# kureta/ddsp-pytorch

Measured on AMD Instinct MI355X. Metric: audio samples/sec/GPU + %HBM-roofline, 16kHz/100-harmonic/batch512, higher is better.
Workload: dtype f32

## Files before the change

ddsp-pytorch_amd/_lib.py:

```python
from __future__ import annotations

import ctypes
import os
import subprocess

_DIR = os.path.dirname(os.path.abspath(__file__))
SO_PATH = os.environ.get("DDSP_HIP_LIB", os.path.join(_DIR, "libddsp_hip.so"))
ABI_VERSION = 5

_lib = None


class DdspHipError(RuntimeError):
    pass


def build(force: bool = False, jobs: int = 4) -> str:
    args = ["make", "-C", os.path.join(_DIR, "csrc"), f"-j{jobs}"]
    if force:
        args.append("-B")
    r = subprocess.run(args, capture_output=True, text=True)
    if r.returncode != 0:
        raise DdspHipError("building libddsp_hip.so failed:\n" + r.stdout[-4000:] + r.stderr[-4000:])
    return SO_PATH


_vp, _i32, _u32, _u64, _long, _size, _f32, _f64 = (ctypes.c_void_p, ctypes.c_int, ctypes.c_uint, ctypes.c_uint64, ctypes.c_long,
                                                   ctypes.c_size_t, ctypes.c_float, ctypes.c_double)

SIGNATURES = {
    "ddsp_hip_abi_version": (_i32, []),
    "ddsp_test_hooks_enabled": (_i32, []),
    "ddsp_osc_scratch_bytes": (_size, [_i32, _i32, _i32]),
    "ddsp_osc_forward_ex": (_i32, [_vp] * 8 + [_i32] * 5 + [_u32, _vp]),
    "ddsp_noise_workspace_bytes": (_size, [_i32, _i32, _i32, _i32]),
    "ddsp_noise_forward_ws": (_i32, [_vp, _vp, _vp, _i32, _i32, _i32, _i32, _u64, _u64, _vp, _i32, _vp, _size, _vp]),
    "ddsp_noise_backward_ws": (_i32, [_vp, _vp, _vp, _i32, _i32, _i32, _i32, _u64, _u64, _vp, _vp, _size, _vp]),
    "ddsp_noise_ola_workspace_bytes": (_size, [_i32, _i32, _i32, _i32]),
    "ddsp_noise_ola_forward": (_i32, [_vp, _vp, _vp, _i32, _i32, _i32, _i32, _u64, _u64, _vp, _i32, _vp, _size, _vp]),
    "ddsp_noise_ola_backward": (_i32, [_vp, _vp, _vp, _i32, _i32, _i32, _i32, _u64, _u64, _vp, _vp, _size, _vp]),
    "ddsp_noise_ola_stream_state_floats": (_size, [_i32]),
    "ddsp_noise_ola_stream": (_i32, [_vp] * 6 + [_i32, _i32, _i32, _i32, _u64, _u64, _vp, _vp, _size, _vp]),
    "ddsp_osc_backward_scratch_bytes": (_size, [_i32, _i32, _i32]),
    "ddsp_osc_backward": (_i32, [_vp] * 8 + [_i32] * 5 + [_vp]),
    "ddsp_osc_set_tiling": (_i32, [_i32]),
    "ddsp_osc_set_path": (_i32, [_i32]),
    "ddsp_osc_plan": (_i32, [_i32] * 5 + [ctypes.POINTER(_i32), _i32]),
    "ddsp_osc_clock": (_i32, [_vp, _i32, _i32, _i32, _i32, _i32, ctypes.POINTER(ctypes.c_double), _vp]),
    "ddsp_noise_set_residency": (_i32, [_i32]),
    "ddsp_noise_get_residency": (_i32, []),
    "ddsp_noise_set_generic": (_i32, [_i32]),
    "ddsp_profile_enable": (_i32, [_i32]),
    "ddsp_profile_select": (_i32, [_u32]),
    "ddsp_profile_read": (_i32, [ctypes.POINTER(_i32), ctypes.POINTER(_f32), _i32]),
    "ddsp_gru_scratch_bytes": (_size, [_i32, _i32]),
    "ddsp_gru_max_batch": (_i32, [_i32, _i32]),
    "ddsp_gru_forward": (_i32, [_vp] * 9 + [_i32] * 3 + [_vp]),
    "ddsp_gru_backward": (_i32, [_vp] * 11 + [_i32] * 3 + [_vp]),
    "ddsp_gru_status": (_i32, [_vp, ctypes.POINTER(_i32)]),
    "ddsp_gru_forward_bf16": (_i32, [_vp] * 9 + [_i32] * 3 + [_vp]),
    "ddsp_gru_backward_bf16": (_i32, [_vp] * 11 + [_i32] * 4 + [_vp]),
    "ddsp_gru_set_mode": (_i32, [_i32]),
    "ddsp_gru_set_fault_step": (_i32, [_i32]),
    "ddsp_outer_ln_lrelu_scratch_bytes": (_size, [_i32]),
    "ddsp_outer_ln_lrelu_forward": (_i32, [_vp] * 8 + [_long, _i32, _f32, _f32, _i32, _vp]),
    "ddsp_outer_ln_lrelu_backward": (_i32, [_vp] * 13 + [_long, _i32, _f32, _i32, _vp]),
    "ddsp_colsum_scratch_bytes": (_size, [_i32]),
    "ddsp_colsum": (_i32, [_vp, _vp, _vp, _long, _i32, _i32, _vp]),
    "ddsp_stft_frames": (_i32, [_vp, _vp, _vp, _long, _long, _i32, _i32, _vp]),
    "ddsp_stft_frames_backward": (_i32, [_vp, _vp, _vp, _long, _long, _i32, _i32, _i32, _vp]),
    "ddsp_mss_scale_scratch_bytes": (_size, []),
    "ddsp_mss_scale_supported": (_i32, [_i32]),
    "ddsp_mss_scale": (_i32, [_vp] * 6 + [_long, _long, _i32, _i32, _f32, _f32, _vp]),
    "ddsp_reverb_impulse": (_i32, [_vp] * 5 + [_i32, _i32, _vp]),
    "ddsp_reverb_impulse_backward": (_i32, [_vp] * 8 + [_i32, _i32, _vp]),
    "ddsp_spectral_mul": (_i32, [_vp, _vp, _vp, _long, _long, _vp]),
    "ddsp_spectral_mul_backward": (_i32, [_vp] * 5 + [_long, _long, _vp]),
    "ddsp_reverb_live_scratch_bytes": (_size, [_i32, _i32]),
    "ddsp_reverb_live": (_i32, [_vp] * 9 + [_i32, _i32, _vp]),
    "ddsp_spectral_loss_scratch_bytes": (_size, []),
    "ddsp_spectral_loss": (_i32, [_vp] * 5 + [_long, _f32, _f32, _vp]),
    "ddsp_scaled_sigmoid_forward": (_i32, [_vp, _vp, _long, _vp]),
    "ddsp_scaled_sigmoid_backward": (_i32, [_vp, _vp, _vp, _long, _vp]),
    "ddsp_heads_sigmoid_forward": (_i32, [_vp] * 4 + [_long, _i32, _i32, _i32, _i32, _vp]),
    "ddsp_heads_sigmoid_backward": (_i32, [_vp] * 5 + [_long, _i32, _i32, _i32, _i32, _vp]),
    "ddsp_ln_lrelu_scratch_bytes": (_size, [_i32]),
    "ddsp_ln_lrelu_forward": (_i32, [_vp] * 6 + [_long, _i32, _f32, _f32, _vp]),
    "ddsp_ln_lrelu_backward": (_i32, [_vp] * 11 + [_long, _i32, _f32, _vp]),
    "ddsp_ln_lrelu_forward_16": (_i32, [_vp] * 6 + [_long, _i32, _f32, _f32, _i32, _vp]),
    "ddsp_ln_lrelu_backward_16": (_i32, [_vp] * 11 + [_long, _i32, _f32, _i32, _vp]),
    "ddsp_resample": (_i32, [_vp] * 4 + [_long, _long, _i32, _i32, _i32, _vp]),
    "ddsp_crepe_frames": (_i32, [_vp] * 3 + [_long, _long, _i32, _long, _vp]),
    "ddsp_crepe_epilogue": (_i32, [_vp] * 7 + [_long, _i32, _i32, _i32, _vp]),
    "ddsp_pitch_decode": (_i32, [_vp] * 8 + [_long, _vp]),
    "ddsp_pitch_centered": (_i32, [_vp] * 6 + [_long, _vp]),
    "ddsp_pitch_viterbi_workspace_bytes": (_size, [_long, _long]),
    "ddsp_pitch_viterbi": (_i32, [_vp] * 6 + [_long, _long, _vp]),
    "ddsp_pitch_voicing_workspace_bytes": (_size, [_long, _long]),
    "ddsp_pitch_voicing": (_i32, [_vp] * 11 + [_long, _long, _i32, _i32, _f32, _f32, _f32, _i32, _vp]),
    "ddsp_yin_salience": (_i32, [_vp] * 3 + [_long, _long, _i32, _long, _vp]),
    "ddsp_harm_workspace_bytes": (_size, [_long, _long, _i32]),
    "ddsp_harm_analysis": (_i32, [_vp] * 7 + [_long, _long, _i32, _i32, _i32, _i32, _vp]),
    "ddsp_harm_resynth": (_i32, [_vp] * 6 + [_long, _long, _i32, _i32, _i32, _u32, _vp]),
    "ddsp_harm_refine_workspace_bytes": (_size, [_long, _long, _i32]),
    "ddsp_harm_refine": (_i32, [_vp] * 8 + [_long, _long, _i32, _i32, _i32, _i32, _f32, _u32, _vp]),
    "ddsp_noise_analysis_workspace_bytes": (_size, [_long, _long, _i32, _i32]),
    "ddsp_noise_analysis": (_i32, [_vp] * 4 + [_long, _long, _i32, _i32, _i32, _i32, _vp]),
    "ddsp_noise_analysis_ola_workspace_bytes": (_size, [_long, _long, _i32, _i32]),
    "ddsp_noise_analysis_ola": (_i32, [_vp] * 4 + [_long, _long, _i32, _i32, _i32, _i32, _vp]),
    "ddsp_transform_controls": (_i32, [_vp] * 11 + [_long, _long, _long, _i32, _i32, _i32, _i32, _vp]),
    "ddsp_morph_controls": (_i32, [_vp] * 17 + [_long, _long, _long, _long, _i32, _i32, _i32, _i32, _i32, _i32, _vp]),
    "ddsp_dtw_workspace_bytes": (_size, [_long, _long, _long]),
    "ddsp_dtw_align": (_i32, [_vp] * 8 + [_size, _long, _long, _long, _i32, _long, _long, _f32, _f64, _vp]),
    "ddsp_loudness_supported": (_i32, [_i32]),
    "ddsp_loudness": (_i32, [_vp] * 3 + [_long, _long, _i32, _i32, _vp]),
    "ddsp_pcm_to_mono": (_i32, [_vp, _vp, _long, _i32, _i32, _vp]),
    "ddsp_make_examples": (_i32, [_vp, _long, _vp, _i32, _long, _long, _long, _long, _i32, _vp, _vp, _vp]),
    "ddsp_griffinlim_supported": (_i32, [_i32]),
    "ddsp_griffinlim_workspace_bytes": (_size, [_long, _long, _i32, _i32]),
    "ddsp_griffinlim": (_i32, [_vp] * 6 + [_size, _long, _long, _i32, _i32, _long, _i32, _f32, _vp]),
    "ddsp_wfft_probe_sizes": (_i32, [_i32, _long, ctypes.POINTER(_long), ctypes.POINTER(_long)]),
    "ddsp_wfft_probe": (_i32, [_i32, _vp, _vp, _long, _vp]),
    "ddsp_griffinlim_stage": (_i32, [_i32] + [_vp] * 8 + [_long, _long, _i32, _i32, _long, _f32, _vp]),
    "ddsp_gather_batch": (_i32, [_vp, _vp, ctypes.POINTER(_long), _i32, _vp, _vp, _long, _long, _i32, _i32, _vp, _vp]),
}
EXPORTS = tuple(SIGNATURES)


def lib():
    global _lib
    if _lib is not None:
        return _lib
    if not os.path.exists(SO_PATH):
        raise DdspHipError(
            f"{SO_PATH} is missing: the DDSP hot path has no CPU fallback. "
            "Build it with `python -c 'import __graft_entry__ as g; g.build()'` or `make -C ddsp-pytorch_amd/csrc`.")
    L = ctypes.CDLL(SO_PATH)
    abi = L.ddsp_hip_abi_version()
    if abi != ABI_VERSION:
        raise DdspHipError(f"{SO_PATH} has ABI {abi}, expected {ABI_VERSION}: rebuild "
                           "(`make -C ddsp-pytorch_amd/csrc` or __graft_entry__.build())")
    for name, (restype, argtypes) in SIGNATURES.items():
        fn = getattr(L, name)
        fn.restype, fn.argtypes = restype, argtypes
    _lib = L
    return L


KERNEL_NAMES = {1: "osc_frame_totals", 2: "osc_scan", 3: "osc_frame_synth", 4: "noise_frame", 5: "noise_impulse_responses"}


def profile_enable(capacity: int, only=None) -> None:
    mask = 0
    for name in only or ():
        mask |= 1 << [k for k, v in KERNEL_NAMES.items() if v == name][0]
    check(lib().ddsp_profile_select(mask), "ddsp_profile_select")
    check(lib().ddsp_profile_enable(capacity), "ddsp_profile_enable")


def profile_read(cap: int = 65536):
    ids = (ctypes.c_int * cap)()
    ms = (ctypes.c_float * cap)()
    n = lib().ddsp_profile_read(ids, ms, cap)
    return [(KERNEL_NAMES.get(ids[i], str(ids[i])), float(ms[i])) for i in range(n)]


def check(rc: int, what: str) -> None:
    if rc == 0:
        return
    if rc == -1:
        raise DdspHipError(f"{what}: invalid argument (DDSP_EINVAL)")
    if rc == -2:
        raise DdspHipError(f"{what}: shape outside the supported range (DDSP_ERANGE)")
    if rc == -3:
        raise DdspHipError(f"{what}: test / tuning hook refused (DDSP_EPERM): set DDSP_TEST_HOOKS=1 before the library is loaded")
    raise DdspHipError(f"{what}: HIP error {rc}")


def osc_plan(B: int, T: int, H: int, hop: int, sample_rate: int) -> dict:
    out = (ctypes.c_int * 8)()
    check(lib().ddsp_osc_plan(B, T, H, hop, sample_rate, out, 8), "ddsp_osc_plan")
    keys = ("harmonics_per_lane", "lanes_per_row", "chunked", "chunk_samples", "chunks_per_row", "row_blocks",
            "compute_units", "workgroups_per_unit")
    return dict(zip(keys, list(out)))


def osc_clock(scratch, B: int, T: int, H: int, hop: int, sample_rate: int, stream: int = 0) -> float:
    ghz = ctypes.c_double(0.0)
    check(lib().ddsp_osc_clock(scratch.data_ptr(), B, T, H, hop, sample_rate, ctypes.byref(ghz), stream or None), "ddsp_osc_clock")
    return float(ghz.value)
```

ddsp-pytorch_amd/csrc/ddsp_noise_wave.hip:

```cpp
#include <hip/hip_runtime.h>
#include <stdint.h>

#include <atomic>

#include "ddsp_hip.h"
#include "ddsp_internal.h"
#include "ddsp_noise_common.h"

using namespace ddsp_noise;

namespace {

typedef float v4f __attribute__((ext_vector_type(4)));

struct Tile { v4f v[5]; };
struct Lines { v4f v[8]; };
struct Pass { float v[16]; };
struct Spectra { v4f e[2], o[2], h64; float z32; };

constexpr int R = kWaveHop;
constexpr int F = kWaveBands;
constexpr int FG = kWaveGroupFrames;
static_assert(R == 128 && F == 65 && FG == 16 && 2 * (F - 1) == R, "the kernel's register and LDS layouts are written for these");
constexpr int KS = 132;
constexpr int XS = 140;
constexpr int kLdsFloats = FG * KS + FG * XS;

#ifndef DDSP_NOISE_ABL
#define DDSP_NOISE_ABL 0
#endif

#ifdef DDSP_NOISE_STAMPS
#define DDSP_STAMP(i) do { asm volatile("s_waitcnt lgkmcnt(0)" ::: "memory"); const unsigned long long now_ = __builtin_amdgcn_s_memtime(); \
                           stamp_sum[i] += now_ - stamp_last; stamp_last = now_; } while (0)
#else
#define DDSP_STAMP(i) do { } while (0)
#endif

template <bool ACC>
__global__ void __launch_bounds__(64, 2) noise_wave_kernel(NoiseParams p, long ngroups)
{
    extern __shared__ __attribute__((aligned(16))) float smem[];
    float *kern = smem;
    float *xs = smem + FG * KS;
    float *Hs = kern, *ys = xs;
    const int lane = threadIdx.x;
#ifdef DDSP_NOISE_STAMPS
    unsigned long long stamp_sum[8] = {0, 0, 0, 0, 0, 0, 0, 0}, stamp_last = __builtin_amdgcn_s_memtime();
    unsigned long long *stamp_out = reinterpret_cast<unsigned long long *>(const_cast<float *>(p.u)) + 8 * blockIdx.x;
    p.u = nullptr;
#endif

    const int mi0 = lane & 15, mq0 = lane >> 4;
    float *ctab = xs;
    ctab[lane] = cospif((float)lane * (1.0f / 64.0f));
    ctab[lane + 64] = cospif((float)(lane + 64) * (1.0f / 64.0f));
    DDSP_WAVE_ORDER();
    Split Be[2], Bo[2];
#pragma unroll
    for (int t = 0; t < 2; ++t) {
        const int n = 16 * t + mi0;
#pragma unroll
        for (int j = 0; j < 8; ++j) {
            const int k = 8 * mq0 + j;
            split3((k == 0 ? 0.5f : 1.0f) * ctab[(2 * k * n) & 127], Be[t], j);
            split3(ctab[((2 * k + 1) * n) & 127], Bo[t], j);
        }
    }
    float w1[2], w2[2];
#pragma unroll
    for (int t = 0; t < 2; ++t) {
        const int n = 16 * t + mi0;
        w1[t] = __fmaf_rn(0.5f, ctab[n], 0.5f) * (1.0f / 64.0f);
        w2[t] = __fmaf_rn(0.5f, ctab[64 - n], 0.5f) * (1.0f / 64.0f);
    }
    DDSP_WAVE_ORDER();
    const uint64_t base_off = p.offset + (p.offset_dev ? *p.offset_dev : 0ull);

    auto load_tile = [&](long g) {
        const v4f *src = reinterpret_cast<const v4f *>(p.Hm + g * FG * F);
        Tile h;
#pragma unroll
        for (int j = 0; j < 4; ++j) h.v[j] = src[lane + 64 * j];
        h.v[4] = src[256 + (lane & 3)];
        return h;
    };

    auto opaque_lane = [&]() { int ln = lane; asm volatile("" : "+v"(ln)); return ln; };

    auto products = [&](const Tile h) {
        const int ln = opaque_lane(), mi = ln & 15, mq = ln >> 4;
#pragma unroll
        for (int j = 0; j < 4; ++j) *reinterpret_cast<v4f *>(Hs + 4 * (ln + 64 * j)) = h.v[j];
        if (ln < 4) *reinterpret_cast<v4f *>(Hs + 4 * (ln + 256)) = h.v[4];
        DDSP_WAVE_ORDER();
        const float *hrow = Hs + mi * F + 16 * mq;
        float hv[16];
#pragma unroll
        for (int j = 0; j < 16; ++j) hv[j] = hrow[j];
        const float h64 = Hs[mi * F + 64];
        Spectra sp;
#pragma unroll
        for (int r = 0; r < 4; ++r) sp.h64[r] = 0.5f * Hs[(4 * mq + r) * F + 64];
        DDSP_WAVE_ORDER();
        Split Ae, Ao;
#pragma unroll
        for (int j = 0; j < 8; ++j) { split3(hv[2 * j], Ae, j); split3(hv[2 * j + 1], Ao, j); }
        v4f (&accE)[2] = sp.e, (&accO)[2] = sp.o;
        accE[0] = accE[1] = accO[0] = accO[1] = (v4f){0, 0, 0, 0};
        constexpr int PA[6] = {2, 1, 0, 1, 0, 0}, PB[6] = {0, 1, 2, 0, 1, 0};
#pragma unroll
        for (int i = 0; i < (DDSP_NOISE_ABL == 3 ? 1 : 6); ++i) {
            accE[0] = __builtin_amdgcn_mfma_f32_16x16x32_bf16(Ae.p[PA[i]], Be[0].p[PB[i]], accE[0], 0, 0, 0);
            accE[1] = __builtin_amdgcn_mfma_f32_16x16x32_bf16(Ae.p[PA[i]], Be[1].p[PB[i]], accE[1], 0, 0, 0);
            accO[0] = __builtin_amdgcn_mfma_f32_16x16x32_bf16(Ao.p[PA[i]], Bo[0].p[PB[i]], accO[0], 0, 0, 0);
            accO[1] = __builtin_amdgcn_mfma_f32_16x16x32_bf16(Ao.p[PA[i]], Bo[1].p[PB[i]], accO[1], 0, 0, 0);
        }
        float t = (mq == 0 ? 0.5f : 1.0f) * hv[0];
#pragma unroll
        for (int j = 1; j < 8; ++j) t += (j & 1) ? -hv[2 * j] : hv[2 * j];
        t += __shfl_xor(t, 16);
        t += __shfl_xor(t, 32);
        sp.z32 = (t + 0.5f * h64) * (0.5f / 64.0f);
        return sp;
    };

    auto taps = [&](const Spectra sp) {
        const int ln = opaque_lane(), mi = ln & 15, mq = ln >> 4;
        const v4f (&accE)[2] = sp.e, (&accO)[2] = sp.o;
        const float z32 = sp.z32;
#pragma unroll
        for (int t = 0; t < 2; ++t) {
            const int n = 16 * t + mi;
#pragma unroll
            for (int r = 0; r < 4; ++r) {
                float *kr = kern + (4 * mq + r) * KS;
                const float ev = accE[t][r] + ((mi & 1) ? -sp.h64[r] : sp.h64[r]);
                const float v1 = (ev + accO[t][r]) * w1[t];
                const float v2 = (ev - accO[t][r]) * w2[t];
                kr[n] = v1;
                if (n != 0) { kr[128 - n] = v1; kr[64 - n] = v2; }
                kr[64 + n] = v2;
            }
        }
        if (mq == 0) { kern[mi * KS + 32] = z32; kern[mi * KS + 96] = z32; }
        DDSP_WAVE_ORDER();
    };

    auto draw = [&](long frame0) {
        const int ln = opaque_lane();
        for (int e = ln; e < FG * 8; e += 64) xs[(e >> 3) * XS + (e & 7)] = 0.0f;
        if (p.u) {
#pragma unroll
            for (int j = 0; j < 8; ++j) {
                const int qi = ln + 64 * j, fr = qi >> 5, q = qi & 31;
                float4 v = *reinterpret_cast<const float4 *>(p.u + (frame0 + fr) * R + 4 * q);
                v.x = v.x * 2.0f - 1.0f; v.y = v.y * 2.0f - 1.0f; v.z = v.z * 2.0f - 1.0f; v.w = v.w * 2.0f - 1.0f;
                *reinterpret_cast<float4 *>(xs + fr * XS + 8 + 4 * q) = v;
            }
        } else {
            const uint64_t c0 = base_off + (uint64_t)frame0 * 32u + (uint64_t)ln;
#pragma unroll
            for (int j = 0; j < 8; ++j) {
                const int qi = ln + 64 * j, fr = qi >> 5, q = qi & 31;
                const uint64_t ctr = c0 + 64u * j;
                uint32_t rr[4];
                if (DDSP_NOISE_ABL == 2) { rr[0] = (uint32_t)ctr; rr[1] = rr[0] * 3u; rr[2] = rr[0] ^ 77u; rr[3] = rr[0] + 5u; }
                else philox4x32_10((uint32_t)ctr, (uint32_t)(ctr >> 32), (uint32_t)p.seed, (uint32_t)(p.seed >> 32), rr);
                float4 v;
                v.x = philox_to_sample(rr[0]); v.y = philox_to_sample(rr[1]); v.z = philox_to_sample(rr[2]); v.w = philox_to_sample(rr[3]);
                *reinterpret_cast<float4 *>(xs + fr * XS + 8 + 4 * q) = v;
            }
        }
        DDSP_WAVE_ORDER();
    };

    auto conv_pass = [&](int pass) {
        const int ln = opaque_lane();
        const int l5 = ln & 31, seg = l5 >> 2;
        const int cf = ((seg >> 1) << 2) | (l5 & 3);
        const int cs = 2 * (ln >> 5) + ((0x96 >> seg) & 1);
        const float *krow = kern + cf * KS;
        const float *xrow = xs + cf * XS + 8;
        const int cA = pass ? 8 + cs : 15 - cs, cB = 15 - cA;
        const int tsw = cA + 1;
        const float *kq_a = krow, *kq_b = krow - 8 * tsw;
        const float *xq_a = xrow + 8 * cA - 8 - 128, *xq_b = xrow + 8 * cB - 8 + 8 * tsw - 128;
        float acc[8], first[8];
#pragma unroll
        for (int u = 0; u < 8; ++u) { acc[u] = 0.0f; first[u] = 0.0f; }
        float4 cur[6], nxt[6];
        auto fetch = [&](float4 (&d)[6], const float *kq, const float *xq, int t) {
            d[0] = *reinterpret_cast<const float4 *>(kq + 8 * t);
            d[1] = *reinterpret_cast<const float4 *>(kq + 8 * t + 4);
            d[2] = *reinterpret_cast<const float4 *>(xq + 8 * (16 - t));
            d[3] = *reinterpret_cast<const float4 *>(xq + 8 * (16 - t) + 4);
            d[4] = *reinterpret_cast<const float4 *>(xq + 8 * (16 - t) + 8);
            d[5] = *reinterpret_cast<const float4 *>(xq + 8 * (16 - t) + 12);
        };
        fetch(cur, kq_a, xq_a, 0);
#pragma unroll
        for (int t = 0; t < (DDSP_NOISE_ABL == 1 ? 1 : 17); ++t) {
            if (t < 16) {
                if (t + 1 < 9) fetch(nxt, kq_a, xq_a, t + 1);
                else { const bool b = t + 1 >= tsw; fetch(nxt, b ? kq_b : kq_a, b ? xq_b : xq_a, t + 1); }
            }
            if (t >= 9 && t == tsw) {
                asm volatile("" ::: "memory");
#pragma unroll
                for (int u = 0; u < 8; ++u) { first[u] = acc[u]; acc[u] = 0.0f; }
            }
            asm volatile("" ::"v"(cur[2].x));
            const float kv[8] = {cur[0].x, cur[0].y, cur[0].z, cur[0].w, cur[1].x, cur[1].y, cur[1].z, cur[1].w};
            const float xw[16] = {cur[2].x, cur[2].y, cur[2].z, cur[2].w, cur[3].x, cur[3].y, cur[3].z, cur[3].w,
                                  cur[4].x, cur[4].y, cur[4].z, cur[4].w, cur[5].x, cur[5].y, cur[5].z, cur[5].w};
#pragma unroll
            for (int v = 0; v < 8; ++v)
#pragma unroll
                for (int u = 0; u < 8; ++u) acc[u] = __fmaf_rn(kv[v], xw[8 + u - v], acc[u]);
#pragma unroll
            for (int e = 0; e < 6; ++e) cur[e] = nxt[e];
            __builtin_amdgcn_sched_barrier(0);
        }
        Pass out;
#pragma unroll
        for (int u = 0; u < 8; ++u) { out.v[u] = first[u]; out.v[8 + u] = acc[u]; }
        return out;
    };

    auto stage = [&](const Pass r0, const Pass r1) {
        const int ln = opaque_lane();
        const int l5 = ln & 31, seg = l5 >> 2;
        const int cf = ((seg >> 1) << 2) | (l5 & 3);
        const int cs = 2 * (ln >> 5) + ((0x96 >> seg) & 1);
        DDSP_WAVE_ORDER();
#pragma unroll
        for (int pass = 0; pass < 2; ++pass) {
            const float (&r)[16] = pass ? r1.v : r0.v;
            const int cA = pass ? 8 + cs : 15 - cs, cB = 15 - cA;
            float *ya = ys + cf * KS + 8 * cA, *yb = ys + cf * KS + 8 * cB;
            *reinterpret_cast<float4 *>(ya) = make_float4(r[0], r[1], r[2], r[3]);
            *reinterpret_cast<float4 *>(ya + 4) = make_float4(r[4], r[5], r[6], r[7]);
            *reinterpret_cast<float4 *>(yb) = make_float4(r[8], r[9], r[10], r[11]);
            *reinterpret_cast<float4 *>(yb + 4) = make_float4(r[12], r[13], r[14], r[15]);
        }
        DDSP_WAVE_ORDER();
    };

    auto read_y = [&](long frame0) {
        const v4f *src = reinterpret_cast<const v4f *>(p.y) + frame0 * (R / 4);
        Lines yv;
#pragma unroll
        for (int j = 0; j < 8; ++j) yv.v[j] = src[lane + 64 * j];
        return yv;
    };
    auto store_y = [&](long frame0, const Lines yv) {
        const int ln = opaque_lane();
        v4f *dst = reinterpret_cast<v4f *>(p.y) + frame0 * (R / 4);
#pragma unroll
        for (int j = 0; j < 8; ++j) {
            const int i4 = ln + 64 * j;
            v4f o = *reinterpret_cast<const v4f *>(ys + (i4 >> 5) * KS + 4 * (i4 & 31));
            if (ACC && DDSP_NOISE_ABL != 4) o += yv.v[j];
            if (DDSP_NOISE_ABL != 4 || o[0] == 123.0f) dst[i4] = o;
        }
        DDSP_WAVE_ORDER();
    };

    long g = blockIdx.x;
    if (g >= ngroups) return;
    Tile hreg = load_tile(g);
    Lines yv;
#pragma unroll
    for (int j = 0; j < 8; ++j) yv.v[j] = (v4f){0.0f, 0.0f, 0.0f, 0.0f};
    taps(products(hreg));
    draw(g * FG);
    DDSP_STAMP(0);
    for (;;) {
        {
            const unsigned slot = (unsigned)__builtin_amdgcn_s_getreg((4 << 0) | (0 << 6) | (3 << 11));
            const unsigned epoch = (unsigned)(__builtin_amdgcn_s_memrealtime() >> 12);
            if ((slot + epoch) & 1u) __builtin_amdgcn_s_setprio(1); else __builtin_amdgcn_s_setprio(0);
        }
        const long frame0 = g * FG;
        const long gn = g + gridDim.x;
        const Pass r0 = conv_pass(0);
        DDSP_STAMP(1);
        hreg = load_tile(gn < ngroups ? gn : g);
        if (ACC && DDSP_NOISE_ABL != 4) yv = read_y(frame0);
        const Pass r1 = conv_pass(1);
        DDSP_STAMP(2);
        stage(r0, r1);
        DDSP_STAMP(3);
        if (gn >= ngroups) break;
        const Spectra sp = products(hreg);
        DDSP_STAMP(4);
        store_y(frame0, yv);
        DDSP_STAMP(5);
        taps(sp);
        DDSP_STAMP(6);
        draw(gn * FG);
        DDSP_STAMP(7);
        g = gn;
    }
    store_y(g * FG, yv);
#ifdef DDSP_NOISE_STAMPS
    DDSP_STAMP(5);
    if (lane == 0)
        for (int i = 0; i < 8; ++i) stamp_out[i] = stamp_sum[i];
#endif
}

constexpr int kDefaultWavesPerCu = 4;
std::atomic<int> g_residency{0};

}

extern "C" int ddsp_noise_set_residency(int waves_per_cu)
{
    if (waves_per_cu < 0 || waves_per_cu > 8) return DDSP_EINVAL;
    g_residency.store(waves_per_cu, std::memory_order_relaxed);
    return 0;
}
extern "C" int ddsp_noise_get_residency(void)
{
    const int v = g_residency.load(std::memory_order_relaxed);
    return v >= 1 && v <= 8 ? v : kDefaultWavesPerCu;
}

namespace ddsp_noise {

hipError_t launch_noise_wave(const NoiseParams &p, long frames, hipStream_t s)
{
    const long ngroups = frames / FG;
    int cus = 0;
    const hipError_t e = ddsp_device_cus(&cus);
    if (e != hipSuccess) return e;
    constexpr size_t lds = sizeof(float) * kLdsFloats;
    const int asked = g_residency.load(std::memory_order_relaxed);
    const long per_cu = asked >= 1 && asked <= 8 ? asked : kDefaultWavesPerCu;
    long resident = ngroups <= (long)cus * 8 ? (long)cus * 8 : (long)cus * per_cu;
    static const long env_waves = [] { const char *ev = getenv("DDSP_NOISE_WAVES"); return (ev && ddsp_hooks_on()) ? atol(ev) : 0L; }();
    if (env_waves > 0 && env_waves <= 8) resident = (long)cus * env_waves;
    const long grid = ngroups < resident ? ngroups : resident;
    const int slot = ddsp_prof::begin(ddsp_prof::NOISE, s);
    if (p.accumulate) hipLaunchKernelGGL(noise_wave_kernel<true>, dim3((unsigned)grid), dim3(64), lds, s, p, ngroups);
    else hipLaunchKernelGGL(noise_wave_kernel<false>, dim3((unsigned)grid), dim3(64), lds, s, p, ngroups);
    ddsp_prof::end(slot, s);
    return hipGetLastError();
}

}
```

include/ddsp_hip.h:

```cpp
#ifndef DDSP_HIP_H
#define DDSP_HIP_H

#include <stddef.h>
#include <stdint.h>

#ifdef __cplusplus
extern "C" {
#endif

#define DDSP_HIP_ABI_VERSION 5

#define DDSP_EINVAL (-1)
#define DDSP_ERANGE (-2)
#define DDSP_EPERM  (-3)

int ddsp_hip_abi_version(void);

int ddsp_test_hooks_enabled(void);

size_t ddsp_osc_scratch_bytes(int B, int T, int H);

#define DDSP_OSC_KEEP_FRAME_SCRATCH 1u
int ddsp_osc_forward_ex(const float *f0, const float *c, const float *a, float *y, void *scratch,
                        const float *live_in, float *live_out, float *dbg_phi,
                        int B, int T, int H, int hop, int sample_rate, unsigned flags, void *stream);

size_t ddsp_noise_workspace_bytes(int B, int T, int F, int hop);
int ddsp_noise_forward_ws(const float *Hmag, const float *uniform, float *y, int B, int T, int F, int hop, uint64_t seed,
                          uint64_t offset, const uint64_t *counter_dev, int accumulate, void *workspace, size_t workspace_bytes,
                          void *stream);
int ddsp_noise_backward_ws(const float *grad_y, const float *uniform, float *grad_H, int B, int T, int F, int hop, uint64_t seed,
                           uint64_t offset, const uint64_t *counter_dev, void *workspace, size_t workspace_bytes, void *stream);

size_t ddsp_noise_ola_workspace_bytes(int B, int T, int F, int hop);
int ddsp_noise_ola_forward(const float *Hmag, const float *uniform, float *y, int B, int T, int F, int hop, uint64_t seed,
                           uint64_t offset, const uint64_t *counter_dev, int accumulate, void *workspace, size_t workspace_bytes,
                           void *stream);
int ddsp_noise_ola_backward(const float *grad_y, const float *uniform, float *grad_H, int B, int T, int F, int hop, uint64_t seed,
                            uint64_t offset, const uint64_t *counter_dev, void *workspace, size_t workspace_bytes, void *stream);

size_t ddsp_noise_ola_stream_state_floats(int F);
int ddsp_noise_ola_stream(const float *Hmag, const float *uniform, const float *dry, float *out, const float *state_in,
                          float *state_out, int B, int T, int F, int hop, uint64_t seed, uint64_t offset, const uint64_t *counter_dev,
                          void *workspace, size_t workspace_bytes, void *stream);

size_t ddsp_osc_backward_scratch_bytes(int B, int T, int H);
int ddsp_osc_backward(const float *grad_y, const float *f0, const float *c, const float *a, const void *fwd_scratch,
                      void *bwd_scratch, float *grad_c, float *grad_a, int B, int T, int H, int hop, int sample_rate,
                      void *stream);

int ddsp_osc_set_tiling(int harmonics_per_lane);
int ddsp_osc_set_path(int path);
int ddsp_osc_plan(int B, int T, int H, int hop, int sample_rate, int *out, int cap);
int ddsp_osc_clock(const void *scratch, int B, int T, int H, int hop, int sample_rate, double *ghz, void *stream);

int ddsp_noise_set_residency(int waves_per_cu);
int ddsp_noise_get_residency(void);

int ddsp_noise_set_generic(int on);

int ddsp_profile_enable(int capacity);
int ddsp_profile_select(unsigned kernel_mask);
int ddsp_profile_read(int *kernel_ids, float *ms, int cap);

size_t ddsp_gru_scratch_bytes(int B, int Hd);
int ddsp_gru_max_batch(int Hd, int backward);
int ddsp_gru_forward(const float *gi, const float *w_hh, const float *b_hh, const float *h0, float *y, float *hT,
                     float *gates, float *hn, void *scratch, int B, int T, int Hd, void *stream);
int ddsp_gru_backward(const float *dy, const float *dhT, const float *w_hh, const float *h0, const float *y,
                      const float *gates, const float *hn, float *d_gi, float *d_gh, float *dh0, void *scratch,
                      int B, int T, int Hd, void *stream);
int ddsp_gru_status(const void *scratch, int *status_host);
int ddsp_gru_forward_bf16(const float *gi, const float *w_hh, const float *b_hh, const float *h0, float *y, float *hT,
                          float *gates, float *hn, void *scratch, int B, int T, int Hd, void *stream);
int ddsp_gru_backward_bf16(const float *dy, const float *dhT, const float *w_hh, const float *h0, const float *y,
                           const float *gates, const float *hn, void *d_gi, void *d_gh, float *dh0, void *scratch,
                           int B, int T, int Hd, int io_type, void *stream);
int ddsp_gru_set_mode(int mode);
int ddsp_gru_set_fault_step(int step);

size_t ddsp_outer_ln_lrelu_scratch_bytes(int D);
int ddsp_outer_ln_lrelu_forward(const float *x, const float *w, const float *bias, const float *gamma, const float *beta, void *y,
                                float *mean, float *rstd, long rows, int D, float eps, float slope, int io_type, void *stream);
int ddsp_outer_ln_lrelu_backward(const void *grad_y, const float *x, const float *w, const float *bias, const void *y,
                                 const float *gamma, const float *mean, const float *rstd, float *grad_w, float *grad_bias,
                                 float *grad_gamma, float *grad_beta, void *scratch, long rows, int D, float slope,
                                 int io_type, void *stream);

size_t ddsp_colsum_scratch_bytes(int N);
int ddsp_colsum(const void *x, float *out, void *scratch, long M, int N, int io_type, void *stream);

int ddsp_stft_frames(const float *x, const float *window, float *frames, long B, long N, int n_fft, int hop, void *stream);
int ddsp_stft_frames_backward(const float *grad_frames, const float *window, float *grad_x, long B, long N, int n_fft, int hop,
                              int accumulate, void *stream);

size_t ddsp_mss_scale_scratch_bytes(void);
int ddsp_mss_scale_supported(int n_fft);
int ddsp_mss_scale(const float *x_pred, const float *x_true, const float *window, float *grad_frames, void *scratch, float *out3,
                   long B, long L, int n_fft, int hop, float alpha, float eps, void *stream);

int ddsp_reverb_impulse(const float *noise, const float *decay, const float *wet, const float *t, float *impulse,
                        int length, int n_out, void *stream);
int ddsp_reverb_impulse_backward(const float *grad_impulse, const float *noise, const float *decay, const float *wet,
                                 const float *t, float *grad_noise, float *grad_decay, float *grad_wet, int length,
                                 int n_used, void *stream);
int ddsp_spectral_mul(const float *x_ri, const float *k_ri, float *y_ri, long rows, long bins, void *stream);
int ddsp_spectral_mul_backward(const float *g_ri, const float *x_ri, const float *k_ri, float *gk_ri, float *s_ri,
                               long rows, long bins, void *stream);
size_t ddsp_reverb_live_scratch_bytes(int length, int n);
int ddsp_reverb_live(const float *x, const float *history_in, float *history_out, const float *noise, const float *decay,
                     const float *wet, const float *t, float *y, void *scratch, int length, int n, void *stream);

size_t ddsp_spectral_loss_scratch_bytes(void);
int ddsp_spectral_loss(const float *pred_ri, const float *true_ri, float *grad_ri, void *scratch, float *out3,
                       long n_bins, float alpha, float eps, void *stream);

int ddsp_scaled_sigmoid_forward(const float *x, float *y, long n, void *stream);
int ddsp_scaled_sigmoid_backward(const float *x, const float *grad_y, float *grad_x, long n, void *stream);
int ddsp_heads_sigmoid_forward(const void *x, float *out0, float *out1, float *out2, long rows, int n0, int n1, int n2,
                               int io_type, void *stream);
int ddsp_heads_sigmoid_backward(const void *x, const float *g0, const float *g1, const float *g2, void *grad_x, long rows,
                                int n0, int n1, int n2, int io_type, void *stream);

size_t ddsp_ln_lrelu_scratch_bytes(int D);
int ddsp_ln_lrelu_forward(const float *x, const float *gamma, const float *beta, float *y, float *mean, float *rstd,
                          long rows, int D, float eps, float slope, void *stream);
int ddsp_ln_lrelu_backward(const float *grad_y, const float *x, const float *y, const float *gamma, const float *mean,
                           const float *rstd, float *grad_x, float *grad_gamma, float *grad_beta, float *grad_xsum, void *scratch,
                           long rows, int D, float slope, void *stream);
#define DDSP_IO_BF16 1
#define DDSP_IO_F16 2
int ddsp_ln_lrelu_forward_16(const void *x, const float *gamma, const float *beta, void *y, float *mean, float *rstd,
                             long rows, int D, float eps, float slope, int io_type, void *stream);
int ddsp_ln_lrelu_backward_16(const void *grad_y, const void *x, const void *y, const float *gamma, const float *mean,
                              const float *rstd, void *grad_x, float *grad_gamma, float *grad_beta, float *grad_xsum, void *scratch,
                              long rows, int D, float slope, int io_type, void *stream);

int ddsp_resample(const float *x, const float *table, const int *first, float *y, long B, long L, int orig, int nw, int ntaps,
                  void *stream);
int ddsp_crepe_frames(const float *y, float *stats, float *frames, long B, long Lr, int hop, long T, void *stream);
int ddsp_crepe_epilogue(const float *conv, const float *bias, const float *running_mean, const float *running_var, const float *gamma,
                        const float *beta, float *out, long N, int C, int Lc, int last, void *stream);
int ddsp_pitch_decode(const float *logits, const float *bias, const float *f0_table, const float *cents_table, float *probs, float *f0,
                      float *harmonicity, float *cents, long N, void *stream);

int ddsp_pitch_centered(const float *probs, const int *center, float *f0, float *harmonicity, float *normalized_cents, int *bins_out,
                        long N, void *stream);
size_t ddsp_pitch_viterbi_workspace_bytes(long B, long T);
int ddsp_pitch_viterbi(const float *probs, const float *log_trans, const float *state_in, float *state_out, int *bins, void *workspace,
                       long B, long T, void *stream);

#define DDSP_VOICING_FILL_NONE 0
#define DDSP_VOICING_FILL_HOLD 1
#define DDSP_VOICING_FILL_INTERPOLATE 2
size_t ddsp_pitch_voicing_workspace_bytes(long B, long T);
int ddsp_pitch_voicing(const float *f0, const float *normalized, const float *periodicity, const float *loudness,
                       const float *state_in, float *f0_out, float *normalized_out, uint8_t *voiced_out, float *periodicity_out,
                       float *state_out, void *workspace, long B, long T, int period_window, int pitch_window, float upper,
                       float lower, float silence, int fill, void *stream);

int ddsp_yin_salience(const float *y, const float *bin_table, float *probs, long B, long Lr, int hop, long T, void *stream);

#define DDSP_HARM_PHASE_READY 1u
size_t ddsp_harm_workspace_bytes(long B, long T, int hop);
int ddsp_harm_analysis(const float *audio, const float *f0, const uint8_t *voiced, float *C, float *a, float *c, void *workspace,
                       long B, long T, int hop, int W, int H, int sample_rate, void *stream);
int ddsp_harm_resynth(const float *C, const float *f0, const float *audio, float *harm, float *resid, void *workspace, long B,
                      long T, int hop, int H, int sample_rate, unsigned flags, void *stream);
size_t ddsp_harm_refine_workspace_bytes(long B, long T, int hop);
int ddsp_harm_refine(const float *audio, const float *f0_in, const float *f0_anchor, const uint8_t *voiced, float *f0_out,
                     float *num_out, float *den_out, void *workspace, long B, long T, int hop, int W, int H, int sample_rate,
                     float max_cents, unsigned flags, void *stream);

size_t ddsp_noise_analysis_workspace_bytes(long B, long T, int F, int hop);
int ddsp_noise_analysis(const float *x, float *H, float *power, void *workspace, long B, long T, int F, int hop, int average,
                        int iterations, void *stream);

size_t ddsp_noise_analysis_ola_workspace_bytes(long B, long T, int F, int hop);
int ddsp_noise_analysis_ola(const float *x, float *H, float *power, void *workspace, long B, long T, int F, int hop, int average,
                            int iterations, void *stream);

int ddsp_transform_controls(const float *f0, const float *a, const float *c, const float *noise, const float *pos, const float *ratio,
                            const float *env, float *f0_out, float *a_out, float *c_out, float *noise_out, long B, long T,
                            long T_out, int H, int H_out, int F, int sample_rate, void *stream);

#define DDSP_MORPH_HZ 0
#define DDSP_MORPH_HARMONIC 1
int ddsp_morph_controls(const float *f0_a, const float *a_a, const float *c_a, const float *noise_a, const float *pos_a,
                        const float *f0_b, const float *a_b, const float *c_b, const float *noise_b, const float *pos_b,
                        const float *mix_f0, const float *mix_amp, const float *mix_noise, float *f0_out, float *a_out, float *c_out,
                        float *noise_out, long B, long T_a, long T_b, long T_out, int H_a, int H_b, int H_out, int F, int sample_rate,
                        int coordinates, void *stream);

size_t ddsp_dtw_workspace_bytes(long B, long T_a, long T_b);
int ddsp_dtw_align(const float *x_a, const float *x_b, float *pos_a, float *pos_b, int *path, int *length, float *cost,
                   void *workspace, size_t workspace_bytes, long B, long T_a, long T_b, int D, long T_out, long radius, float penalty,
                   double timing, void *stream);

int ddsp_loudness_supported(int n_fft);
int ddsp_loudness(const float *x, const double *a_weight, float *out, long B, long L, int n_fft, int hop, void *stream);

#define DDSP_PCM_S16 1
#define DDSP_PCM_S32 2
#define DDSP_PCM_F32 3
int ddsp_pcm_to_mono(const void *pcm, float *y, long L, int C, int format, void *stream);
int ddsp_make_examples(const float *y, long y_len, const long *files, int n_files, long e0, long E, long duration, long step, int p,
                       float *enc_in, float *audio, void *stream);


int ddsp_griffinlim_supported(int n_fft);
size_t ddsp_griffinlim_workspace_bytes(long B, long T, int n_fft, int with_angles);
int ddsp_griffinlim(const float *mag, const float *angles, const float *window, const float *env, float *y, void *workspace,
                    size_t workspace_bytes, long B, long T, int n_fft, int hop, long L, int n_iter, float c, void *stream);

#define DDSP_WFFT_PAIR_FWD 0
#define DDSP_WFFT_PAIR_INV 5
#define DDSP_WFFT_WAVE8_FWD 10
#define DDSP_WFFT_WAVE8_INV 11
#define DDSP_WFFT_WAVE8_HALFZERO 12
#define DDSP_WFFT_WAVE16_FWD 13
#define DDSP_WFFT_WAVE16_INV 14
#define DDSP_WFFT_WAVE16_HALFZERO 15
#define DDSP_WFFT_REAL2048_FWD 16
#define DDSP_WFFT_REAL2048_INV 17
#define DDSP_WFFT_TWIDDLES 18
#define DDSP_WFFT_SCALE 19
#define DDSP_WFFT_WAVEMAX 20
#define DDSP_WFFT_TWIDDLE_COUNT 88
int ddsp_wfft_probe_sizes(int form, long units, long *in_floats, long *out_floats);
int ddsp_wfft_probe(int form, const float *in, float *out, long units, void *stream);

#define DDSP_GL_STAGE_SYNTH 0
#define DDSP_GL_STAGE_OVERLAP 1
#define DDSP_GL_STAGE_ANALYSIS 2
int ddsp_griffinlim_stage(int stage, const float *S, const float *ang0, const float *R, const float *Rprev, const float *in,
                          const float *window, const float *env, float *out, long B, long T, int n_fft, int hop, long L, float c,
                          void *stream);

#define DDSP_GATHER_MAX_ARRAYS 8
#define DDSP_GATHER_BAD_INDEX 1
#define DDSP_GATHER_BAD_CURSOR 2
int ddsp_gather_batch(const void **src, void **dst, const long *row_floats, int n_arrays, const long *perm, long *cursor,
                      long perm_len, long n_examples, int rows, int advance, unsigned *error, void *stream);

#ifdef __cplusplus
}
#endif
#endif
```

Baseline: 30.97 billion.

## Run noise filter circular convolution on 4x4x1 f32 MFMA instead of scalar FMAs

Replaces the scalar-FMA two-pass circular convolution in the noise wave kernel with a matrix-core formulation using mfma_f32_4x4x1f32. The filter taps and noise samples get new padded, plane-split LDS layouts so each lane can fetch operands without bank conflicts, and the two passes accumulate into one 8-window accumulator that is staged with vector stores. The intent is to offload the FMA-bound convolution to the matrix units. In exchange it adds LDS padding, zeroing stores and a different operand schedule, and it ships a hook-gated probe kernel for checking correctness.

Measured after the change: 31.30 billion, median of 6. +1.1%, better.

```diff
diff --git a/ddsp-pytorch_amd/_lib.py b/ddsp-pytorch_amd/_lib.py
--- a/ddsp-pytorch_amd/_lib.py
+++ b/ddsp-pytorch_amd/_lib.py
@@ -49,6 +49,7 @@
     "ddsp_osc_clock": (_i32, [_vp, _i32, _i32, _i32, _i32, _i32, ctypes.POINTER(ctypes.c_double), _vp]),
     "ddsp_noise_set_residency": (_i32, [_i32]),
     "ddsp_noise_get_residency": (_i32, []),
+    "ddsp_noise_conv_probe": (_i32, [_vp, _vp, _vp, _vp]),
     "ddsp_noise_set_generic": (_i32, [_i32]),
     "ddsp_profile_enable": (_i32, [_i32]),
     "ddsp_profile_select": (_i32, [_u32]),
diff --git a/ddsp-pytorch_amd/csrc/ddsp_noise_conv_plan.h b/ddsp-pytorch_amd/csrc/ddsp_noise_conv_plan.h
--- /dev/null
+++ b/ddsp-pytorch_amd/csrc/ddsp_noise_conv_plan.h
@@ -0,0 +1,40 @@
+#pragma once
+
+namespace ddsp_noise {
+namespace conv {
+
+constexpr int kFrames = 16;
+constexpr int kSamples = 128;
+constexpr int kWindow = 16;
+constexpr int kWindows = kSamples / kWindow;
+constexpr int kMu = 16;
+constexpr int kOperands = 8;
+constexpr int kStepsPerMu = kOperands * (kOperands + 1) / 2;
+constexpr int kSteps = kMu * kStepsPerMu;
+
+constexpr int a_first(int mu) { return mu >= 13 ? -1 : 0; }
+constexpr int beta_first(int mu) { return mu >= 13 ? 1 : 0; }
+constexpr int window_of(int r, int s) { return r + s; }
+constexpr int tap_base(int mu, int a) { return 16 * a + mu; }
+constexpr int src_base(int mu, int beta) { return 16 * beta - mu; }
+
+constexpr int kTapPad = 4;
+constexpr int kTapStride = kTapPad + kSamples;
+constexpr int kTapFloats = kFrames * kTapStride;
+constexpr int tap_slot(int b, int m) { return b * kTapStride + kTapPad + m; }
+constexpr int tap_offset(int mu, int a) { return kTapPad + tap_base(mu, a); }
+
+constexpr int kSrcPad = 16;
+constexpr int kSrcRow = (kSrcPad + kSamples) / 4;
+constexpr int kSrcPlane = kFrames * kSrcRow;
+constexpr int kSrcFloats = 4 * kSrcPlane;
+constexpr int src_slot(int b, int p) { return (p & 3) * kSrcPlane + b * kSrcRow + ((p + kSrcPad) >> 2); }
+constexpr int src_offset(int mu, int beta) { return src_slot(0, src_base(mu, beta)); }
+
+static_assert(kTapStride % 32 == 4 && kSrcRow % 32 == 4, "bank-conflict-free operand reads");
+static_assert(kTapStride % 4 == 0 && kSrcRow % 4 == 0 && kSrcPlane % 4 == 0, "16-byte aligned rows");
+static_assert(tap_base(13, a_first(13)) == -3 && tap_offset(13, a_first(13)) >= 0, "the first step reads inside the tap padding");
+static_assert(src_base(12, beta_first(12)) == -12 && kSrcPad + src_base(12, 0) >= 0, "the lowest source sample is inside the padding");
+
+}
+}
diff --git a/ddsp-pytorch_amd/csrc/ddsp_noise_wave.hip b/ddsp-pytorch_amd/csrc/ddsp_noise_wave.hip
--- a/ddsp-pytorch_amd/csrc/ddsp_noise_wave.hip
+++ b/ddsp-pytorch_amd/csrc/ddsp_noise_wave.hip
@@ -6,6 +6,7 @@
 #include "ddsp_hip.h"
 #include "ddsp_internal.h"
 #include "ddsp_noise_common.h"
+#include "ddsp_noise_conv_plan.h"
 
 using namespace ddsp_noise;
 
@@ -15,16 +16,18 @@
 
 struct Tile { v4f v[5]; };
 struct Lines { v4f v[8]; };
-struct Pass { float v[16]; };
+struct Acc { v4f d[8]; };
 struct Spectra { v4f e[2], o[2], h64; float z32; };
 
 constexpr int R = kWaveHop;
 constexpr int F = kWaveBands;
 constexpr int FG = kWaveGroupFrames;
 static_assert(R == 128 && F == 65 && FG == 16 && 2 * (F - 1) == R, "the kernel's register and LDS layouts are written for these");
-constexpr int KS = 132;
-constexpr int XS = 140;
-constexpr int kLdsFloats = FG * KS + FG * XS;
+namespace cp = ddsp_noise::conv;
+constexpr int KS = cp::kTapStride;
+constexpr int KP = cp::kTapPad;
+static_assert(cp::kFrames == FG && cp::kSamples == R && cp::kSrcFloats >= FG * KS, "the staging tile lies over the noise tile");
+constexpr int kLdsFloats = cp::kTapFloats + cp::kSrcFloats;
 
 #ifndef DDSP_NOISE_ABL
 #define DDSP_NOISE_ABL 0
@@ -37,12 +40,52 @@
 #define DDSP_STAMP(i) do { } while (0)
 #endif
 
+__device__ __forceinline__ Acc conv_half(const float *kern, const float *xs, int ln, int mu0, Acc acc)
+{
+    const int b = ln >> 2, q = ln & 3;
+    const float *ka = kern + b * cp::kTapStride + q;
+    const float *xb = xs + b * cp::kSrcRow + q;
+    float A[cp::kOperands], B[cp::kOperands], An[cp::kOperands], Bn[cp::kOperands];
+    auto fetch = [&](float (&a)[cp::kOperands], float (&bb)[cp::kOperands], int mu) {
+#pragma unroll
+        for (int r = 0; r < cp::kOperands; ++r) {
+            a[r] = ka[cp::tap_offset(mu, cp::a_first(mu) + r)];
+            bb[r] = xb[cp::src_offset(mu, cp::beta_first(mu) + r)];
+        }
+    };
+    fetch(A, B, mu0);
+#pragma unroll
+    for (int m = 0; m < (DDSP_NOISE_ABL == 1 ? 1 : cp::kMu / 2); ++m) {
+        if (m + 1 < cp::kMu / 2) fetch(An, Bn, mu0 + m + 1);
+#pragma unroll
+        for (int r = 0; r < cp::kOperands; ++r)
+#pragma unroll
+            for (int s = cp::kOperands - 1 - r; s >= 0; --s)
+                acc.d[cp::window_of(r, s)] = __builtin_amdgcn_mfma_f32_4x4x1f32(A[r], B[s], acc.d[cp::window_of(r, s)], 0, 0, 0);
+        __builtin_amdgcn_sched_group_barrier(0x100, 2 * cp::kOperands, 0);
+        __builtin_amdgcn_sched_group_barrier(0x008, cp::kStepsPerMu, 0);
+        if (m + 1 < cp::kMu / 2) {
+#pragma unroll
+            for (int r = 0; r < cp::kOperands; ++r) { A[r] = An[r]; B[r] = Bn[r]; }
+        }
+        __builtin_amdgcn_sched_barrier(0);
+    }
+    return acc;
+}
+
+__device__ __forceinline__ void stage_acc(float *ys, int ln, const Acc acc)
+{
+    float *row = ys + (ln >> 2) * KS + 4 * (ln & 3);
+#pragma unroll
+    for (int o = 0; o < cp::kWindows; ++o) *reinterpret_cast<v4f *>(row + cp::kWindow * o) = acc.d[o];
+}
+
 template <bool ACC>
 __global__ void __launch_bounds__(64, 2) noise_wave_kernel(NoiseParams p, long ngroups)
 {
     extern __shared__ __attribute__((aligned(16))) float smem[];
     float *kern = smem;
-    float *xs = smem + FG * KS;
+    float *xs = smem + cp::kTapFloats;
     float *Hs = kern, *ys = xs;
     const int lane = threadIdx.x;
 #ifdef DDSP_NOISE_STAMPS
@@ -127,6 +170,7 @@
 
     auto taps = [&](const Spectra sp) {
         const int ln = opaque_lane(), mi = ln & 15, mq = ln >> 4;
+        kern[(ln >> 2) * KS + (ln & 3)] = 0.0f;
         const v4f (&accE)[2] = sp.e, (&accO)[2] = sp.o;
         const float z32 = sp.z32;
 #pragma unroll
@@ -134,7 +178,7 @@
             const int n = 16 * t + mi;
 #pragma unroll
             for (int r = 0; r < 4; ++r) {
-                float *kr = kern + (4 * mq + r) * KS;
+                float *kr = kern + (4 * mq + r) * KS + KP;
                 const float ev = accE[t][r] + ((mi & 1) ? -sp.h64[r] : sp.h64[r]);
                 const float v1 = (ev + accO[t][r]) * w1[t];
                 const float v2 = (ev - accO[t][r]) * w2[t];
@@ -143,20 +187,24 @@
                 kr[64 + n] = v2;
             }
         }
-        if (mq == 0) { kern[mi * KS + 32] = z32; kern[mi * KS + 96] = z32; }
-        DDSP_WAVE_ORDER();
-    };
-
+        if (mq == 0) { kern[mi * KS + KP + 32] = z32; kern[mi * KS + KP + 96] = z32; }
+        DDSP_WAVE_ORDER();
+    };
+
+    auto put = [&](int fr, int q, const float4 v) {
+        float *d = xs + cp::src_slot(fr, 0) + q;
+        d[0] = v.x; d[cp::kSrcPlane] = v.y; d[2 * cp::kSrcPlane] = v.z; d[3 * cp::kSrcPlane] = v.w;
+    };
     auto draw = [&](long frame0) {
         const int ln = opaque_lane();
-        for (int e = ln; e < FG * 8; e += 64) xs[(e >> 3) * XS + (e & 7)] = 0.0f;
+        *reinterpret_cast<v4f *>(xs + (ln >> 4) * cp::kSrcPlane + (ln & 15) * cp::kSrcRow) = (v4f){0.0f, 0.0f, 0.0f, 0.0f};
         if (p.u) {
 #pragma unroll
             for (int j = 0; j < 8; ++j) {
                 const int qi = ln + 64 * j, fr = qi >> 5, q = qi & 31;
                 float4 v = *reinterpret_cast<const float4 *>(p.u + (frame0 + fr) * R + 4 * q);
                 v.x = v.x * 2.0f - 1.0f; v.y = v.y * 2.0f - 1.0f; v.z = v.z * 2.0f - 1.0f; v.w = v.w * 2.0f - 1.0f;
-                *reinterpret_cast<float4 *>(xs + fr * XS + 8 + 4 * q) = v;
+                put(fr, q, v);
             }
         } else {
             const uint64_t c0 = base_off + (uint64_t)frame0 * 32u + (uint64_t)ln;
@@ -169,81 +217,16 @@
                 else philox4x32_10((uint32_t)ctr, (uint32_t)(ctr >> 32), (uint32_t)p.seed, (uint32_t)(p.seed >> 32), rr);
                 float4 v;
                 v.x = philox_to_sample(rr[0]); v.y = philox_to_sample(rr[1]); v.z = philox_to_sample(rr[2]); v.w = philox_to_sample(rr[3]);
-                *reinterpret_cast<float4 *>(xs + fr * XS + 8 + 4 * q) = v;
+                put(fr, q, v);
             }
         }
         DDSP_WAVE_ORDER();
     };
 
-    auto conv_pass = [&](int pass) {
-        const int ln = opaque_lane();
-        const int l5 = ln & 31, seg = l5 >> 2;
-        const int cf = ((seg >> 1) << 2) | (l5 & 3);
-        const int cs = 2 * (ln >> 5) + ((0x96 >> seg) & 1);
-        const float *krow = kern + cf * KS;
-        const float *xrow = xs + cf * XS + 8;
-        const int cA = pass ? 8 + cs : 15 - cs, cB = 15 - cA;
-        const int tsw = cA + 1;
-        const float *kq_a = krow, *kq_b = krow - 8 * tsw;
-        const float *xq_a = xrow + 8 * cA - 8 - 128, *xq_b = xrow + 8 * cB - 8 + 8 * tsw - 128;
-        float acc[8], first[8];
-#pragma unroll
-        for (int u = 0; u < 8; ++u) { acc[u] = 0.0f; first[u] = 0.0f; }
-        float4 cur[6], nxt[6];
-        auto fetch = [&](float4 (&d)[6], const float *kq, const float *xq, int t) {
-            d[0] = *reinterpret_cast<const float4 *>(kq + 8 * t);
-            d[1] = *reinterpret_cast<const float4 *>(kq + 8 * t + 4);
-            d[2] = *reinterpret_cast<const float4 *>(xq + 8 * (16 - t));
-            d[3] = *reinterpret_cast<const float4 *>(xq + 8 * (16 - t) + 4);
-            d[4] = *reinterpret_cast<const float4 *>(xq + 8 * (16 - t) + 8);
-            d[5] = *reinterpret_cast<const float4 *>(xq + 8 * (16 - t) + 12);
-        };
-        fetch(cur, kq_a, xq_a, 0);
-#pragma unroll
-        for (int t = 0; t < (DDSP_NOISE_ABL == 1 ? 1 : 17); ++t) {
-            if (t < 16) {
-                if (t + 1 < 9) fetch(nxt, kq_a, xq_a, t + 1);
-                else { const bool b = t + 1 >= tsw; fetch(nxt, b ? kq_b : kq_a, b ? xq_b : xq_a, t + 1); }
-            }
-            if (t >= 9 && t == tsw) {
-                asm volatile("" ::: "memory");
-#pragma unroll
-                for (int u = 0; u < 8; ++u) { first[u] = acc[u]; acc[u] = 0.0f; }
-            }
-            asm volatile("" ::"v"(cur[2].x));
-            const float kv[8] = {cur[0].x, cur[0].y, cur[0].z, cur[0].w, cur[1].x, cur[1].y, cur[1].z, cur[1].w};
-            const float xw[16] = {cur[2].x, cur[2].y, cur[2].z, cur[2].w, cur[3].x, cur[3].y, cur[3].z, cur[3].w,
-                                  cur[4].x, cur[4].y, cur[4].z, cur[4].w, cur[5].x, cur[5].y, cur[5].z, cur[5].w};
-#pragma unroll
-            for (int v = 0; v < 8; ++v)
-#pragma unroll
-                for (int u = 0; u < 8; ++u) acc[u] = __fmaf_rn(kv[v], xw[8 + u - v], acc[u]);
-#pragma unroll
-            for (int e = 0; e < 6; ++e) cur[e] = nxt[e];
-            __builtin_amdgcn_sched_barrier(0);
-        }
-        Pass out;
-#pragma unroll
-        for (int u = 0; u < 8; ++u) { out.v[u] = first[u]; out.v[8 + u] = acc[u]; }
-        return out;
-    };
-
-    auto stage = [&](const Pass r0, const Pass r1) {
-        const int ln = opaque_lane();
-        const int l5 = ln & 31, seg = l5 >> 2;
-        const int cf = ((seg >> 1) << 2) | (l5 & 3);
-        const int cs = 2 * (ln >> 5) + ((0x96 >> seg) & 1);
-        DDSP_WAVE_ORDER();
-#pragma unroll
-        for (int pass = 0; pass < 2; ++pass) {
-            const float (&r)[16] = pass ? r1.v : r0.v;
-            const int cA = pass ? 8 + cs : 15 - cs, cB = 15 - cA;
-            float *ya = ys + cf * KS + 8 * cA, *yb = ys + cf * KS + 8 * cB;
-            *reinterpret_cast<float4 *>(ya) = make_float4(r[0], r[1], r[2], r[3]);
-            *reinterpret_cast<float4 *>(ya + 4) = make_float4(r[4], r[5], r[6], r[7]);
-            *reinterpret_cast<float4 *>(yb) = make_float4(r[8], r[9], r[10], r[11]);
-            *reinterpret_cast<float4 *>(yb + 4) = make_float4(r[12], r[13], r[14], r[15]);
-        }
+    auto conv = [&](int half, const Acc acc) { return conv_half(kern, xs, opaque_lane(), half * (cp::kMu / 2), acc); };
+    auto stage = [&](const Acc acc) {
+        DDSP_WAVE_ORDER();
+        stage_acc(ys, opaque_lane(), acc);
         DDSP_WAVE_ORDER();
     };
 
@@ -284,13 +267,16 @@
         }
         const long frame0 = g * FG;
         const long gn = g + gridDim.x;
-        const Pass r0 = conv_pass(0);
+        Acc acc;
+#pragma unroll
+        for (int o = 0; o < cp::kWindows; ++o) acc.d[o] = (v4f){0.0f, 0.0f, 0.0f, 0.0f};
+        acc = conv(0, acc);
         DDSP_STAMP(1);
         hreg = load_tile(gn < ngroups ? gn : g);
         if (ACC && DDSP_NOISE_ABL != 4) yv = read_y(frame0);
-        const Pass r1 = conv_pass(1);
+        acc = conv(1, acc);
         DDSP_STAMP(2);
-        stage(r0, r1);
+        stage(acc);
         DDSP_STAMP(3);
         if (gn >= ngroups) break;
         const Spectra sp = products(hreg);
@@ -311,6 +297,29 @@
 #endif
 }
 
+__global__ void __launch_bounds__(64) noise_conv_probe_kernel(const float *__restrict__ k, const float *__restrict__ x, float *__restrict__ y)
+{
+    __shared__ __attribute__((aligned(16))) float smem[kLdsFloats];
+    float *kern = smem, *xs = smem + cp::kTapFloats;
+    const int lane = threadIdx.x;
+    for (int e = lane; e < kLdsFloats; e += 64) smem[e] = 0.0f;
+    DDSP_WAVE_ORDER();
+    for (int e = lane; e < FG * R; e += 64) {
+        kern[cp::tap_slot(e / R, e % R)] = k[e];
+        xs[cp::src_slot(e / R, e % R)] = x[e];
+    }
+    DDSP_WAVE_ORDER();
+    Acc acc;
+#pragma unroll
+    for (int o = 0; o < cp::kWindows; ++o) acc.d[o] = (v4f){0.0f, 0.0f, 0.0f, 0.0f};
+    acc = conv_half(kern, xs, lane, 0, acc);
+    acc = conv_half(kern, xs, lane, cp::kMu / 2, acc);
+    DDSP_WAVE_ORDER();
+    stage_acc(xs, lane, acc);
+    DDSP_WAVE_ORDER();
+    for (int e = lane; e < FG * R; e += 64) y[e] = xs[(e / R) * KS + e % R];
+}
+
 constexpr int kDefaultWavesPerCu = 4;
 std::atomic<int> g_residency{0};
 
@@ -326,6 +335,14 @@
 {
     const int v = g_residency.load(std::memory_order_relaxed);
     return v >= 1 && v <= 8 ? v : kDefaultWavesPerCu;
+}
+
+extern "C" int ddsp_noise_conv_probe(const float *k, const float *x, float *y, void *stream)
+{
+    if (!ddsp_hooks_on()) return DDSP_EPERM;
+    if (!k || !x || !y) return DDSP_EINVAL;
+    hipLaunchKernelGGL(noise_conv_probe_kernel, dim3(1), dim3(64), 0, (hipStream_t)stream, k, x, y);
+    return (int)hipGetLastError();
 }
 
 namespace ddsp_noise {
diff --git a/include/ddsp_hip.h b/include/ddsp_hip.h
--- a/include/ddsp_hip.h
+++ b/include/ddsp_hip.h
@@ -56,6 +56,7 @@
 
 int ddsp_noise_set_residency(int waves_per_cu);
 int ddsp_noise_get_residency(void);
+int ddsp_noise_conv_probe(const float *k, const float *x, float *y, void *stream);
 
 int ddsp_noise_set_generic(int on);
 
```
